# mikeferguson/ndt_2d

Measured on AMD Instinct MI355X. Metric: pose-candidates x beams scored per second, higher is better.
Workload: dtype f64

## Files before the change

experiments/asm_loop_mix.py:

```python
#!/usr/bin/env python3
import collections
import hashlib
import json
import os
import re
import subprocess
import sys
import tempfile

R = os.path.dirname(os.path.dirname(os.path.abspath(__file__)))
KERNELS = [
    ("ndt2d_match_lane.hip", "match_lane_compact_kernel", r"25match_lane_compact_kernelENS"),
    ("ndt2d_match_lane.hip", "match_lane_compact_parts_kernel", r"31match_lane_compact_parts_kernelENS"),
    ("ndt2d_match_small.hip", "match_small_kernel", r"18match_small_kernelILb1ELb1ELb1EEE"),
    ("ndt2d_poses_compact.hip", "score_poses_compact_kernel", r"26score_poses_compact_kernelILi256ELb1ELb1ELb0EEE"),
]


def kernel_lines(path, pattern):
    out, on = [], False
    for line in open(path):
        if not on:
            if re.match(r"^_Z\w*%s\w*:" % pattern, line):
                on = True
            continue
        out.append(line)
        if line.strip().startswith("s_endpgm"):
            break
    return out


def loop_depths(lines):
    label_at = {}
    for i, line in enumerate(lines):
        m = re.match(r"^(\.LBB\d+_\d+):", line)
        if m:
            label_at[m.group(1)] = i
    depth = [0] * len(lines)
    for i, line in enumerate(lines):
        m = re.match(r"^\s+s_c?branch\w*\s+(\.LBB\d+_\d+)", line)
        if m:
            j = label_at.get(m.group(1))
            if j is not None and j <= i:
                for k in range(j, i + 1):
                    depth[k] += 1
# ... 122 lines not shown
```

experiments/lane_paths.py:

```python
#!/usr/bin/env python3
import json
import os
import sys

ROOT = os.path.dirname(os.path.dirname(os.path.abspath(__file__)))
sys.path.insert(0, ROOT)
import torch
from ndt_2d_amd import ScanMatcherNDT, synth, _capi

cfg = int(sys.argv[1]) if len(sys.argv) > 1 else 2
m = ScanMatcherNDT(0)
m.initialize("paths", **synth.matcher_params(cfg))
m.addScans(synth.map_scans(cfg))
guess, pts, _ = synth.query_scan(cfg)
n_th, n_lin, n_b = m.prepare_search(guess, pts)
if cfg == 4:
    n_th_run = (n_th + 7) // 8
    launch = lambda ptr: m.match_launch_strided(0, 8, n_th_run, scores_ptr=ptr)
else:
    n_th_run = n_th
    launch = lambda ptr: m.match_launch(0, n_th, scores_ptr=ptr)
hist = torch.zeros(256, dtype=torch.float64, device="cuda")
launch(hist.data_ptr())
m.synchronize()
hist.zero_()
torch.cuda.synchronize()
launch(hist.data_ptr())
m.synchronize()
h = hist.cpu().numpy()
names = ["items", "chunks_pretested", "beams_in_lookup_groups", "groups_with_a_live_lane", "beams_with_a_live_lane",
         "exact_evaluations", "evaluations_by_reference_index", "evaluations_with_exp", "skip_refreshes",
         "items_reduced", "single_beams"]
p1 = (n_lin + 7) // 8
out = {"what": "path counts of one search, wave-level events (experiments/lane_paths.py, -DNDT2D_LANE_PATHS build)",
       "cfg": cfg, "variant": m.last_variant(), "n_theta_run": n_th_run, "n_lin": n_lin, "beams": n_b,
       "wave_beams": n_th_run * p1 * p1 * n_b, "units": n_th_run * n_lin * n_lin * n_b,
       "build_info": _capi.build_info(),
       "counts": {n: float(h[200 + i]) for i, n in enumerate(names)}}
print(json.dumps(out, indent=1))
```

ndt_2d_amd/csrc/device/ndt2d_context.h:

```cpp
#ifndef NDT2D_CONTEXT_H_
#define NDT2D_CONTEXT_H_

#include <hip/hip_runtime.h>

#include <atomic>
#include <cmath>
#include <cstring>
#include <string>
#include <utility>
#include <vector>

#include "ndt2d_guard.h"
#include "ndt2d_hip.h"
#include "ndt2d_kernels.h"

#pragma GCC visibility push(hidden)

struct DeviceBuffer
{
  double * ptr = nullptr;
  size_t cap = 0;
  DeviceBuffer() = default;
  DeviceBuffer(const DeviceBuffer &) = delete;
  DeviceBuffer & operator=(const DeviceBuffer &) = delete;
// ... 48 lines not shown
  DeviceBuffer coarse_bits;
  int coarse_log2 = -1;
  DeviceBuffer block_bytes;
  int block_bytes_log2 = -1;
  uint32_t sparse_n = 0;
  const uint32_t * sparse_index = nullptr;
  const double * sparse_cells6 = nullptr;
  DeviceBuffer b_points, b_scans, b_offsets, b_world, b_keys, b_vals, b_temp, b_seg;
  std::vector<double> stage_scans;
  std::vector<uint32_t> stage_offsets;
  std::vector<uint32_t> stage_seen;

  DeviceBuffer beams;
  size_t n_beams = 0;
  PinnedStage stage_beams, stage_tables, stage_grid, stage_call;
  const double * beams_ptr = nullptr;
  const double * tables_ptr = nullptr;
  DeviceBuffer call_dev;

  uint64_t queued = 0, reached = 0;
  uint64_t match_pos = 0, few_pos = 0;
  double * host_res = nullptr;
  double * host_res_dev = nullptr;
  unsigned long long seq = 0;
  unsigned long long match_seq = 0;
  unsigned long long * done_words = nullptr;

  DeviceBuffer tables;
  bool tables_uploaded = false;
  size_t n_th = 0, n_lin = 0;
  double pose_x = 0.0, pose_y = 0.0;
  double dlin_absmax = 0.0;
  double patch_span = -1.0;
  double beam_rmax = 0.0;
  bool has_search = false;

  DeviceBuffer ws_match, ws_poses, record, stats, outer;
  DeviceBuffer tmp_scores, tmp_poses, tmp_noise;
  hipStream_t up_stream = nullptr, down_stream = nullptr;
  hipEvent_t pipe_up[NDT2D_PIPELINE_PIECES] = {}, pipe_scored[NDT2D_PIPELINE_PIECES] = {}, pipe_idle = nullptr;
  DeviceBuffer piece_stats;
  int pipeline_pieces = 0;
  int last_pieces = 1;
  DeviceBuffer near_list;
  DeviceBuffer scan_ranges, scan_points, scan_info;
  size_t n_scan_points = 0;

  hipEvent_t ring0[NDT2D_TIMING_HISTORY] = {}, ring1[NDT2D_TIMING_HISTORY] = {};
  uint64_t n_timed_launches = 0;
  hipEvent_t ev0 = nullptr, ev1 = nullptr;
  bool timing = true;
  bool timed = false;
  int last_kernels = 0;
  const char * last_variant = "";
  int force_variant = ndt2d::kVariantAuto;
  bool batched_only = false;
  int eigen_form = 0;

  bool match_pending = false;
  uint64_t match_launches = 0, match_fetches = 0;
  bool few_pending = false;
  unsigned long long few_seq = 0;
  size_t few_n_poses = 0;
  bool few_stats = false;
  bool sums_pending = false;
  unsigned long long sums_seq = 0;
// ... 251 lines not shown
```

ndt_2d_amd/csrc/device/ndt2d_context_search.hip:

```cpp
#include <algorithm>
#include <limits>

#include "device/ndt2d_context.h"

using namespace ndt2d_device;

namespace
{

void lattice_extent(ndt2d_context * h, const double * dlin, size_t n_lin)
{
  h->dlin_absmax = 0.0;
  h->patch_span = 0.0;
  for (size_t i = 0; i < n_lin; ++i)
  {
    if (std::fabs(dlin[i]) > h->dlin_absmax) h->dlin_absmax = std::fabs(dlin[i]);
  }
  for (size_t i = 0; i < n_lin && h->patch_span >= 0.0; i += 8)
  {
    const size_t last = i + 7 < n_lin ? i + 7 : n_lin - 1;
    for (size_t k = i; k < last; ++k)
    {
      if (!(dlin[k + 1] >= dlin[k])) h->patch_span = -1.0;
    }
    if (h->patch_span >= 0.0 && dlin[last] - dlin[i] > h->patch_span) h->patch_span = dlin[last] - dlin[i];
  }
}

}

double ndt2d_device::beam_reach(const double * beams_xy, size_t n_beams)
{
  double rmax = 0.0;
  for (size_t i = 0; i < n_beams; ++i)
  {
    const double r = std::hypot(beams_xy[2 * i], beams_xy[2 * i + 1]);
    if (r > rmax) rmax = r;
    if (std::isnan(r)) rmax = std::numeric_limits<double>::infinity();
  }
  return rmax;
}

extern "C" {

int ndt2d_set_beams(ndt2d_handle h, const double * beams_xy, size_t n_beams)
{
  NDT2D_C_TRY
  if (h == nullptr) return NDT2D_ERR_INVALID;
  if (beams_xy == nullptr || n_beams == 0 || n_beams > (1u << 20))
  {
    return fail(h, NDT2D_ERR_INVALID, "ndt2d_set_beams: bad argument");
  }
  NDT2D_HIP(h, hipSetDevice(h->device));
  int rc = ensure(h, h->beams, 2 * n_beams + 2);
  if (rc != NDT2D_OK) return rc;
  rc = stage_acquire(h, h->stage_beams, 2 * n_beams);
  if (rc != NDT2D_OK) return rc;
  std::memcpy(h->stage_beams.ptr, beams_xy, 2 * n_beams * sizeof(double));
  rc = stage_submit(h, h->stage_beams, h->beams.ptr, 2 * n_beams);
// ... 108 lines not shown
  if (h == nullptr) return NDT2D_ERR_INVALID;
  if (!h->has_grid) return fail(h, NDT2D_ERR_NO_GRID, "ndt2d_match_launch: no grid");
  if (!h->has_search || h->n_beams == 0)
  {
    return fail(h, NDT2D_ERR_STATE, "ndt2d_match_launch: set_beams/set_search first");
  }
  if (th_count == 0 || th_stride == 0 || th_first >= h->n_th ||
      (th_count - 1) > (h->n_th - 1 - th_first) / th_stride)
  {
    return fail(h, NDT2D_ERR_INVALID, "ndt2d_match_launch: bad theta range");
  }
  const size_t th_begin = th_first, th_end = th_first + th_count;
  NDT2D_TEST_MAYBE_FAIL(h, "ndt2d_match_launch");
  NDT2D_HIP(h, hipSetDevice(h->device));
  int rc = ensure(h, h->record, NDT2D_MATCH_RECORD_DOUBLES);
  if (rc != NDT2D_OK) return rc;
  if (h->bytes_job.n > 0)
  {
    hipError_t be = ndt2d::launch_sparse_bytes(h->grid, h->bytes_job, h->stream);
    if (be != hipSuccess) return fail_hip(h, be, "launch_sparse_bytes");
    h->bytes_job.n = 0;
  }

  ndt2d::MatchArgs a{};
  a.grid = h->grid;
  a.beams_xy = h->beams_ptr;
  a.n_beams = static_cast<uint32_t>(h->n_beams);
  a.dth = h->tables_ptr;
  a.cos_th = h->tables_ptr + h->n_th;
  a.sin_th = h->tables_ptr + 2 * h->n_th;
  a.dlin = h->tables_ptr + 3 * h->n_th;
  a.dlin_absmax = h->dlin_absmax;
  a.patch_span = h->patch_span;
  a.beam_rmax = h->beam_rmax;
  a.n_th = static_cast<uint32_t>(h->n_th);
  a.n_lin = static_cast<uint32_t>(h->n_lin);
  a.th_begin = static_cast<uint32_t>(th_begin);
  a.th_end = static_cast<uint32_t>(th_end);
  a.th_stride = static_cast<uint32_t>(th_stride);
  a.pose_x = h->pose_x;
  a.pose_y = h->pose_y;
  a.scores = d_scores;
  if (!(h->force_variant & (ndt2d::kVariantWave | ndt2d::kVariantLane)))
  {
    const int k = ndt2d::match_small_block_log2(a, ndt2d::poses_lds_per_block());
    if (k > 0)
    {
      if (h->block_bytes_log2 != k)
      {
        rc = ensure(h, h->block_bytes, ndt2d::grid_block_bytes_size(h->grid, static_cast<uint32_t>(k)) / 8 + 2);
        if (rc != NDT2D_OK) return rc;
        hipError_t be = ndt2d::grid_block_bytes_launch(h->grid, static_cast<uint32_t>(k),
                                                       reinterpret_cast<uint8_t *>(h->block_bytes.ptr), h->stream);
        if (be != hipSuccess) return fail_hip(h, be, "grid_block_bytes_launch");
        h->block_bytes_log2 = k;
      }
      a.grid.block_bytes = reinterpret_cast<const uint8_t *>(h->block_bytes.ptr);
      a.grid.block_bytes_log2 = static_cast<uint32_t>(k);
    }
  }
  if (!h->tables_uploaded)
  {
    a.host_tables = h->stage_tables.ptr;
    if (ndt2d::match_needs_device_tables(a, !(h->force_variant & ndt2d::kVariantWave), h->force_variant))
    {
      rc = stage_submit(h, h->stage_tables, h->tables.ptr, 3 * h->n_th + h->n_lin);
// ... 168 lines not shown
```

ndt_2d_amd/csrc/ndt2d_kernels.h:

```cpp
#ifndef NDT2D_KERNELS_H_
#define NDT2D_KERNELS_H_

#include <hip/hip_runtime.h>
#include <math.h>
#include <stddef.h>
#include <stdint.h>

inline void ndt2d_cos_sin(double t, double * c, double * s)
{
  sincos(t, s, c);
}

namespace ndt2d
{

constexpr int kCellDoubles = 6;
constexpr int kCellStrideGlobal = 8;

struct GridDesc
{
  const double * cells_lds_image;
  const double * cells_global;
  const uint32_t * occ_bits;
  const uint8_t * cell_bytes;
  const double * compact_records;
  const uint16_t * cell_rank;
  uint32_t n_occ;
  const uint8_t * block_bytes;
  uint32_t block_bytes_log2;
  uint32_t size_x, size_y, ncell;
  double cell_size;
  double inv_cell_size;
  int pow2;
  double origin_x, origin_y;
};

struct MatchArgs
{
  GridDesc grid;
  const double * beams_xy;
  uint32_t n_beams;
  const double * dth;
  const double * cos_th;
  const double * sin_th;
  const double * dlin;
  double dlin_absmax;
  double beam_rmax;
  double patch_span;
  uint32_t n_th, n_lin;
  uint32_t th_begin, th_end;
  uint32_t th_stride;
  double pose_x, pose_y;
  double * scores;
  const double * host_tables;
  uint32_t beam_parts, part_beams;
  double * part_sums;
  double * partials;
  uint32_t * next_item;
  uint32_t chunk;
};

struct PosesArgs
{
  GridDesc grid;
  const double * beams_xy;
  uint32_t n_beams;
  const double * poses_xyt;
  uint64_t n_poses;
  double * scores;
  double * partials;
  double beam_rmax;
  float screen_guard;
  const uint32_t * coarse_bits;
  uint32_t coarse_log2;
};

struct BuildArgs
{
  GridDesc grid;
  const double * points_xy;
  uint32_t n_points;
// ... 215 lines not shown
```

ndt_2d_amd/csrc/ndt2d_lane_fn.h:

```cpp
#ifndef NDT2D_LANE_FN_H_
#define NDT2D_LANE_FN_H_

#include <cmath>

#include "ndt2d_device_fn.h"

namespace ndt2d
{

namespace
{

constexpr int kPatch = 8;
#ifndef NDT2D_LANE_UNROLL
#define NDT2D_LANE_UNROLL 8
#endif
constexpr int kUnroll = NDT2D_LANE_UNROLL;
constexpr double kFracScale = 65536.0;
constexpr int kMapStride = 256;
constexpr int kMaxMapCells = 256;
constexpr uint32_t kNearUnits = 4;
constexpr double kBoxMargin = 1.0 / 1024.0;
constexpr double kTwo24 = 16777216.0;
constexpr double kTwo52 = 4503599627370496.0;
constexpr double kNearBias = kNearUnits * (kTwo24 + 1.0);
static_assert(kNearUnits == 4, "near_boundary() tests the biased fraction against 2 * kNearUnits");

struct LaneGeom
{
  int32_t pad;
  int32_t sub_log2;
  int32_t block_log2;
  double unit_scale;
  double inv_scaled;
  int32_t map_h;
  int32_t win_x0, win_y0, win_w, win_h;
  double k_min, k_max_x, k_max_y;
  int32_t no_skip;
  int32_t box_span;
};

constexpr int kMaxBoxSpan = 3;
constexpr int kMaxBlockLog2 = 3;

__device__ __forceinline__ double exponent_upper_bound(const double * rec, double x0, double x1,
                                                       double y0, double y1)
{
  const double mx = rec[0], my = rec[1], h00 = rec[2], h01 = rec[3], h11 = rec[4];
  if (!(h00 < 0.0 && h11 < 0.0 && h00 * h11 - h01 * h01 > 0.0)) return HUGE_VAL;
  const double a0 = x0 - mx, a1 = x1 - mx, b0 = y0 - my, b1 = y1 - my;
  double best;
  if (a0 <= 0.0 && a1 >= 0.0 && b0 <= 0.0 && b1 >= 0.0)
  {
    best = 0.0;
  }
  else
  {
    best = -HUGE_VAL;
    const double qa[2] = {a0, a1}, qb[2] = {b0, b1};
#pragma unroll
    for (int k = 0; k < 2; ++k)
    {
      double q0 = qa[k];
      double q1 = fmin(fmax(-h01 * q0 / h11, b0), b1);
      best = fmax(best, h00 * q0 * q0 + 2.0 * h01 * q0 * q1 + h11 * q1 * q1);
      q1 = qb[k];
      q0 = fmin(fmax(-h01 * q1 / h00, a0), a1);
      best = fmax(best, h00 * q0 * q0 + 2.0 * h01 * q0 * q1 + h11 * q1 * q1);
    }
  }
  const double am = fmax(fabs(a0), fabs(a1)), bm = fmax(fabs(b0), fabs(b1));
  const double magnitude = fabs(h00) * am * am + 2.0 * fabs(h01) * am * bm + fabs(h11) * bm * bm;
  return best + (1e-9 * magnitude + 1e-6);
}

// ... 179 lines not shown
__device__ __forceinline__ uint64_t near_boundary(uint32_t v)
{
  uint64_t lanes;
  asm("v_cmp_gt_u16_e64 %0, 8, %1" : "=s"(lanes) : "v"(v));
  return lanes;
}

__device__ __forceinline__ uint2 lds_two_dwords_at(uint32_t address)
{
  typedef const __attribute__((address_space(3), aligned(4))) uint32_t * lds_u32_ptr;
  const lds_u32_ptr p = reinterpret_cast<lds_u32_ptr>(address);
  return make_uint2(p[0], p[1]);
}

__device__ __forceinline__ bool patch_can_score(double s, int32_t span)
{
  const uint32_t lo = static_cast<uint32_t>(__double2loint(s));
  const uint32_t hi = static_cast<uint32_t>(__double2hiint(s));
  const uint32_t address = __builtin_amdgcn_perm(hi, lo, 0x0c0c0502u);
  const uint32_t base = address & ~3u;
  const uint32_t shift = address & 3u;
  uint32_t any = 0;
#pragma unroll
  for (int r = 0; r <= kMaxBoxSpan; ++r)
  {
    if (r <= span)
    {
      const uint2 w = lds_two_dwords_at(base + static_cast<uint32_t>(r) * kMapStride);
      any |= __builtin_amdgcn_alignbyte(w.y, w.x, shift);
    }
  }
  const uint32_t columns = span >= 3 ? 0xfcfcfcfcu : (0xfcfcfcfcu >> (8 * (3 - span)));
  return (any & columns) != 0u;
}

__device__ __forceinline__ double lds_record_exponent(uint32_t cells_address, uint32_t idx,
                                                      double px, double py)
{
  typedef const __attribute__((address_space(3), aligned(16))) double * lds_double_ptr;
  const lds_double_ptr rec = reinterpret_cast<lds_double_ptr>(
    __umul24(idx, static_cast<uint32_t>(kCellDoubles * sizeof(double))) + cells_address);
  return record_exponent(rec[0], rec[1], rec[2], rec[3], rec[4], px, py);
}

struct SkipState
{
  double skip_below;
  uint32_t skip_level;
};

__device__ __forceinline__ SkipState skip_state(double sum, int32_t no_skip)
{
  SkipState s;
  if (no_skip)
  {
    s.skip_below = -HUGE_VAL;
    s.skip_level = 0;
    return s;
  }
  s.skip_below = negligible_below(sum);
  const int32_t l = static_cast<int32_t>(ceil(s.skip_below)) + 63;
  s.skip_level = static_cast<uint32_t>(min(max(l, 1), 63)) << 2;
  return s;
}

template <int U, bool POW2, bool LDS_RECORDS, bool SCALAR_ROWS = true, bool COMPACT = false>
// ... 145 lines not shown
  }
  if (coarse_map && block_log2 > 0)
  {
    const int32_t cells = 1 << block_log2;
    geo->win_w += geo->win_x0 & (cells - 1);
    geo->win_h += geo->win_y0 & (cells - 1);
    geo->win_x0 &= ~(cells - 1);
    geo->win_y0 &= ~(cells - 1);
  }
  geo->pad = pad;
  geo->block_log2 = block_log2;
  const size_t grid_bytes = static_cast<size_t>(args.grid.ncell + 1) * kCellDoubles * sizeof(double);
  const bool records_fit = grid_bytes + kMapStride * need_h <= lds_per_block;
  const uint64_t p1 = (args.n_lin + kPatch - 1) / kPatch;
  const bool small_search = static_cast<uint64_t>(args.n_th) * p1 * p1 < 4096;
  int sub_log2 = (small_search || coarse_map || block_log2 > 0) ? 0 : 2;
  for (; sub_log2 > 0; --sub_log2)
  {
    const uint64_t w = need_w << sub_log2, h = need_h << sub_log2;
    if (w > kMaxMapCells || h > kMaxMapCells) continue;
    const size_t bytes = static_cast<size_t>(kMapStride) * h + (records_fit ? grid_bytes : 0);
    if (bytes <= lds_per_block) break;
  }
  geo->sub_log2 = sub_log2;
  geo->unit_scale = kFracScale * static_cast<double>(1 << sub_log2) / static_cast<double>(1 << block_log2);
  geo->inv_scaled = args.grid.inv_cell_size * geo->unit_scale;
  geo->map_h = static_cast<int32_t>((need_h << sub_log2) >> block_log2);
  const double reach_units = (lin_cells + 1.0) * geo->unit_scale;
  geo->k_min = reach_units;
  geo->k_max_x = static_cast<double>(need_w - 1) * geo->unit_scale - reach_units;
  geo->k_max_y = static_cast<double>(need_h - 1) * geo->unit_scale - reach_units;
  *map_bytes = static_cast<size_t>(kMapStride) * geo->map_h;
  geo->box_span = -1;
  if (args.patch_span >= 0.0)
  {
    const double span_units = std::ceil(args.patch_span * args.grid.inv_cell_size * geo->unit_scale) + 2.0;
    const double sub_cells = std::floor((65535.0 + span_units) / 65536.0);
    if (sub_cells <= static_cast<double>(kMaxBoxSpan)) geo->box_span = static_cast<int32_t>(sub_cells);
  }
  return true;
}

}

}

#endif
```

ndt_2d_amd/csrc/ndt2d_match_lane.hip:

```cpp
#include <cmath>
#include <cstdlib>

#include <type_traits>

#include "ndt2d_lane_fn.h"

namespace ndt2d
{

namespace
{

constexpr uint32_t kDynamicItemsFromBeams = 256;
constexpr int kLaneThreads = 1024;
constexpr int kLaneThreadsSmall = 256;
#ifndef NDT2D_LANE_THREADS_COMPACT
#define NDT2D_LANE_THREADS_COMPACT 768
#endif
constexpr int kLaneThreadsCompact = NDT2D_LANE_THREADS_COMPACT;
#define NDT2D_LANE_COMPACT_WAVES_PER_EU (NDT2D_LANE_THREADS_COMPACT / 128)

__global__ void __launch_bounds__(256) outer_table_kernel(const MatchArgs a, double4 * outer,
                                                          uint8_t * map_out, const LaneGeom geo)
{
// ... 11 lines not shown
        continue;
      }
      const int32_t sub = 1 << geo.sub_log2;
      const int32_t cx = (mx >> geo.sub_log2) - geo.pad + geo.win_x0;
      const int32_t cy = (my >> geo.sub_log2) - geo.pad + geo.win_y0;
      map_out[i] = sub_cell_byte(g, cx, cy, mx & (sub - 1), my & (sub - 1), geo.sub_log2);
    }
  }

  if (blockIdx.x == 0 && threadIdx.x < kItemShards) a.next_item[threadIdx.x * kItemShardStride] = 0u;
  const uint64_t n = static_cast<uint64_t>(a.th_end - a.th_begin) * a.n_beams;
  for (uint64_t i = static_cast<uint64_t>(blockIdx.x) * 256 + threadIdx.x; i < n;
       i += static_cast<uint64_t>(gridDim.x) * 256)
  {
    const uint32_t t = static_cast<uint32_t>(i / a.n_beams);
    const uint32_t b = static_cast<uint32_t>(i - static_cast<uint64_t>(t) * a.n_beams);
    const uint32_t ith = a.th_begin + t * a.th_stride;
    const double ct = a.cos_th[ith];
    const double st = a.sin_th[ith];
    const double2 p = reinterpret_cast<const double2 *>(a.beams_xy)[b];
    double4 o;
    o.x = p.x * ct - p.y * st + a.pose_x;
    o.y = p.x * st + p.y * ct + a.pose_y;
    double kx = ((o.x - a.grid.origin_x) * a.grid.inv_cell_size + (geo.pad - geo.win_x0)) * geo.unit_scale;
    double ky = ((o.y - a.grid.origin_y) * a.grid.inv_cell_size + (geo.pad - geo.win_y0)) * geo.unit_scale;
    kx = !(kx >= geo.k_min) ? geo.k_min : (kx > geo.k_max_x ? geo.k_max_x : kx);
    ky = !(ky >= geo.k_min) ? geo.k_min : (ky > geo.k_max_y ? geo.k_max_y : ky);
    o.z = kTwo52 + (rint(ky) * kTwo24 + rint(kx)) + kNearBias;
    o.w = 0.0;
    outer[i] = o;
  }
}

__device__ __forceinline__ void item_place(uint32_t item, uint32_t patches, uint32_t patches_1d,
                                           uint32_t th_mid, uint32_t & t, uint32_t & pxi, uint32_t & pyi)
{
  const uint32_t rank = item / patches;
  const uint32_t p = item - rank * patches;
  t = (rank & 1u) ? th_mid + (rank + 1u) / 2u : th_mid - rank / 2u;
  pxi = p / patches_1d;
  pyi = p - pxi * patches_1d;
}

__device__ __forceinline__ double packed_offset(double dx, double dy, double inv_scaled)
{
  return rint(dy * inv_scaled) * kTwo24 + rint(dx * inv_scaled);
}

__device__ __forceinline__ double no_index_here()
{
  static_assert(kNoIndex == 1.0e308, "the literal below is 1.0e308");
  uint32_t lo, hi;
  asm volatile("v_mov_b32 %0, 0x85ebc8a0\n\tv_mov_b32 %1, 0x7fe1ccf3" : "=v"(lo), "=v"(hi));
  return __hiloint2double(static_cast<int>(hi), static_cast<int>(lo));
}

template <int THREADS, bool POW2, bool LDS_RECORDS, bool DYNAMIC_ITEMS, bool COMPACT, bool PARTS = false>
__device__ __forceinline__ void match_lane_body(
  const MatchArgs & a, const double4 * __restrict__ outer, const uint8_t * __restrict__ map_image,
  const LaneGeom & geo)
{
  extern __shared__ __align__(16) double lds[];
  const GridDesc & g = a.grid;
#if defined(NDT2D_LANE_HIST) || defined(NDT2D_LANE_PATHS)
  if (blockIdx.x == 0 && threadIdx.x == 0) g_lane_hist = a.scores;
#endif
  uint8_t * lds_map = reinterpret_cast<uint8_t *>(lds);
  const uint32_t map_bytes = static_cast<uint32_t>(geo.map_h) * kMapStride;
  const uint32_t rank_bytes = COMPACT ? compact_rank_bytes(g.ncell) : 0u;
  double * lds_cells = lds + (map_bytes + rank_bytes) / sizeof(double);

  if (COMPACT)
  {
    const uint4 * src_rank = reinterpret_cast<const uint4 *>(g.cell_rank);
    uint4 * dst_rank = reinterpret_cast<uint4 *>(lds_map + map_bytes + kRankLead);
    for (uint32_t i = threadIdx.x; i < (rank_bytes - kRankLead) / 16; i += THREADS) dst_rank[i] = src_rank[i];
    if (threadIdx.x == 0)
    {
      reinterpret_cast<uint16_t *>(lds_map + map_bytes + kRankLead)[-1] = static_cast<uint16_t>(g.n_occ);
    }
    const uint32_t n2 = (g.n_occ + 1) * kCellDoubles / 2;
    const double2 * src = reinterpret_cast<const double2 *>(g.compact_records);
    double2 * dst = reinterpret_cast<double2 *>(lds_cells);
    for (uint32_t i = threadIdx.x; i < n2; i += THREADS) dst[i] = src[i];
  }
  else if (LDS_RECORDS)
  {
    stage_grid_to_lds(g, lds_cells);
  }
  {
    const uint32_t n16 = static_cast<uint32_t>(kMapStride) * geo.map_h / 16;
    const uint4 * src = reinterpret_cast<const uint4 *>(map_image);
    uint4 * dst = reinterpret_cast<uint4 *>(lds_map);
    for (uint32_t i = threadIdx.x; i < n16; i += THREADS) dst[i] = src[i];
  }
  __syncthreads();

#ifdef NDT2D_LANE_TRACE
  const unsigned long long trace_t0 = wall_clock64();
  unsigned long long trace_last = trace_t0, trace_max = 0, trace_last_start = trace_t0;
  uint32_t trace_items = 0, trace_prev_item = 0, trace_flagged = 0;
#endif
  LaneCtx c;
  c.rank_address = map_bytes + (COMPACT ? kRankLead : 0u);
  c.lds_cells_address = map_bytes + rank_bytes;
  c.sub_log2 = static_cast<uint32_t>(geo.sub_log2);
  c.exact_index = geo.block_log2 > 0 ? 1u : 0u;
  c.idx_bias = static_cast<uint32_t>(geo.pad - geo.win_y0) * g.size_x +
               static_cast<uint32_t>(geo.pad - geo.win_x0);
  c.size_x = g.size_x;

  const uint32_t lane = threadIdx.x & (kWave - 1);
  const uint32_t wave = __builtin_amdgcn_readfirstlane(threadIdx.x >> 6);
  const uint32_t n_lin = a.n_lin;
  const uint32_t patches_1d = (n_lin + kPatch - 1) / kPatch;
  const uint32_t patches = patches_1d * patches_1d;
  const uint32_t n_items = (a.th_end - a.th_begin) * patches * (PARTS ? a.beam_parts : 1u);
  constexpr uint32_t kLaneWaves = THREADS / kWave;
  const uint32_t n_workers = gridDim.x * kLaneWaves;
  const uint32_t worker = wave * gridDim.x + blockIdx.x;
  const uint64_t per_theta = static_cast<uint64_t>(n_lin) * n_lin;
  const uint32_t th_mid = (a.th_end - a.th_begin - 1u) / 2u;
  const uint32_t home_shard = blockIdx.x % kItemShards;
  const double inv_scaled = geo.inv_scaled;

  double best_s = 0.0;
  double best_i = kNoIndex;
  double acc[10];
#pragma unroll
  for (int k = 0; k < 10; ++k) acc[k] = 0.0;
  for (uint32_t item = worker; item < n_items;)
  {
    uint32_t t, pxi, pyi;
#ifdef NDT2D_LANE_TRACE
    {
      const unsigned long long now = wall_clock64();
      if (trace_items > 0 && now - trace_last > trace_max) trace_max = now - trace_last;
      if (trace_items > 0 && a.scores != nullptr && lane == 0)
      {
        a.scores[5 * 8192 + 150000 + trace_prev_item] = static_cast<double>(now - trace_last);
        a.scores[5 * 8192 + 300000 + trace_prev_item] = static_cast<double>(trace_flagged);
      }
      trace_flagged = 0;
      trace_prev_item = item;
      trace_last = now;
      trace_last_start = now;
      ++trace_items;
      if (a.scores != nullptr && lane == 0) a.scores[5 * 8192 + item] = static_cast<double>(now);
    }
#endif
    const uint32_t whole_item = PARTS ? item / a.beam_parts : item;
    const uint32_t part = PARTS ? item - whole_item * a.beam_parts : 0u;
    item_place(whole_item, patches, patches_1d, th_mid, t, pxi, pyi);
    uint32_t lane_here = lane;
    asm volatile("" : "+v"(lane_here));
    const uint32_t ix = pxi * kPatch + (lane_here >> 3);
    const uint32_t iy = pyi * kPatch + (lane_here & 7);
    const double dx = a.dlin[min(ix, n_lin - 1)];
    const double dy = a.dlin[min(iy, n_lin - 1)];
    const double dxy = packed_offset(dx, dy, inv_scaled);
    const double4 * __restrict__ row = outer + static_cast<size_t>(t) * a.n_beams;

    double sum = 0.0;
    SkipState skip = skip_state(0.0, geo.no_skip);
    NDT2D_PATH(200, 1);
    const double dxy_corner = __hiloint2double(__builtin_amdgcn_readfirstlane(__double2hiint(dxy)),
                                               __builtin_amdgcn_readfirstlane(__double2loint(dxy)));
    const uint32_t beams_begin = PARTS ? part * a.part_beams : 0u;
    const uint32_t beams_end = PARTS ? min(beams_begin + a.part_beams, a.n_beams) : a.n_beams;
    for (uint32_t b0 = beams_begin; b0 < beams_end; b0 += kWave)
    {
      uint64_t can_score = ~0ull;
      if (geo.box_span >= 0)
      {
        const double k = row[min(b0 + lane, a.n_beams - 1u)].z;
        can_score = __builtin_amdgcn_ballot_w64(patch_can_score(k + dxy_corner, geo.box_span));
        NDT2D_PATH(201, 1);
      }
#ifdef NDT2D_LANE_TRACE
      trace_flagged += static_cast<uint32_t>(__popcll(can_score));
#endif
      const uint32_t chunk_end = min(b0 + static_cast<uint32_t>(kWave), beams_end);
      uint32_t b = b0;
      for (; b + kUnroll <= chunk_end; b += kUnroll, can_score >>= kUnroll)
      {
        if ((can_score & ((1ull << kUnroll) - 1ull)) == 0ull) continue;
        double4 o[kUnroll];
#pragma unroll
        for (int u = 0; u < kUnroll; ++u) o[u] = row[b + u];
        __builtin_amdgcn_s_setprio(3);
        lane_beams<kUnroll, POW2, LDS_RECORDS, true, COMPACT>(g, c, o, dx, dy, dxy, sum, skip, geo.no_skip);
        __builtin_amdgcn_s_setprio(0);
      }
      for (; b < chunk_end; ++b, can_score >>= 1)
      {
        if ((can_score & 1ull) == 0ull) continue;
        const double4 one[1] = {row[b]};
        lane_beams<1, POW2, LDS_RECORDS, true, COMPACT>(g, c, one, dx, dy, dxy, sum, skip, geo.no_skip);
      }
    }

    if (PARTS)
    {
      a.part_sums[static_cast<size_t>(item) * kWave + lane] = sum;
      uint32_t next = n_items;
      if (lane == kWave - 1)
      {
        for (uint32_t tried = 0; tried < kItemShards && next >= n_items; ++tried)
        {
          const uint32_t shard = (home_shard + tried) % kItemShards;
          const uint32_t k = atomicAdd(a.next_item + shard * kItemShardStride, 1u);
          const uint64_t candidate = static_cast<uint64_t>(n_workers) + static_cast<uint64_t>(k) * kItemShards + shard;
          if (candidate < n_items) next = static_cast<uint32_t>(candidate);
        }
      }
      item = static_cast<uint32_t>(__builtin_amdgcn_readlane(static_cast<int>(next), kWave - 1));
      continue;
    }
    uint32_t lane_again = lane;
    asm volatile("" : "+v"(lane_again));
    const uint32_t ix_e = pxi * kPatch + (lane_again >> 3);
    const uint32_t iy_e = pyi * kPatch + (lane_again & 7);
    if ((ix_e < n_lin) & (iy_e < n_lin))
    {
      const uint32_t ix = ix_e, iy = iy_e;
      const double score = -sum;
      const uint64_t local = static_cast<uint64_t>(t) * per_theta + static_cast<uint64_t>(ix) * n_lin + iy;
      const double flat = static_cast<double>(
        static_cast<uint64_t>(a.th_begin + t * a.th_stride) * per_theta + static_cast<uint64_t>(ix) * n_lin + iy);
      if (DYNAMIC_ITEMS)
      {
        if (score < best_s)
        {
          best_s = score;
          best_i = flat;
        }
      }
      else if (score < 0.0)
      {
        merge_best(score, flat, best_s, best_i);
      }
      const double dt = a.dth[a.th_begin + t * a.th_stride];
      acc[0] += (dx * dx) * score;
      acc[1] += (dx * dy) * score;
      acc[2] += (dx * dt) * score;
      acc[3] += (dy * dy) * score;
      acc[4] += (dy * dt) * score;
      acc[5] += (dt * dt) * score;
      acc[6] += dx * score;
      acc[7] += dy * score;
      acc[8] += dt * score;
      acc[9] += score;
#if !defined(NDT2D_LANE_HIST) && !defined(NDT2D_LANE_TRACE) && !defined(NDT2D_LANE_PATHS)
      if (a.scores != nullptr) a.scores[local] = score;
#endif
    }
// ... 33 lines not shown
#pragma unroll
    for (int k = 0; k < 10; ++k) acc[k] = 0.0;
  }
#ifdef NDT2D_LANE_TRACE
  if (a.scores != nullptr && lane == 0)
  {
    const unsigned long long now = wall_clock64();
    if (trace_items > 0 && now - trace_last > trace_max) trace_max = now - trace_last;
    if (trace_items > 0) a.scores[5 * 8192 + 150000 + trace_prev_item] = static_cast<double>(now - trace_last);
    if (trace_items > 0) a.scores[5 * 8192 + 300000 + trace_prev_item] = static_cast<double>(trace_flagged);
    a.scores[5 * worker] = static_cast<double>(trace_t0);
    a.scores[5 * worker + 1] = static_cast<double>(now);
    a.scores[5 * worker + 2] = static_cast<double>(trace_items);
    a.scores[5 * worker + 3] = static_cast<double>(trace_max);
    a.scores[5 * worker + 4] = static_cast<double>(trace_last_start);
  }
#endif
  if (!DYNAMIC_ITEMS)
  {
    wave_best_to_last_lane(best_s, best_i);
#pragma unroll
    for (int k = 0; k < 10; ++k) acc[k] = wave_sum_to_last_lane(acc[k]);
    if (lane == kWave - 1)
    {
      double * out = a.partials + static_cast<size_t>(worker) * kRecord;
      out[0] = best_s;
      out[1] = best_i;
#pragma unroll
      for (int k = 0; k < 10; ++k) out[2 + k] = acc[k];
    }
  }
}

template <int THREADS, bool POW2, bool LDS_RECORDS, bool DYNAMIC_ITEMS>
__global__ void __launch_bounds__(THREADS) match_lane_kernel(
  const MatchArgs a, const double4 * __restrict__ outer, const uint8_t * __restrict__ map_image,
  const LaneGeom geo)
{
  match_lane_body<THREADS, POW2, LDS_RECORDS, DYNAMIC_ITEMS, false>(a, outer, map_image, geo);
}

__global__ void __launch_bounds__(kLaneThreadsCompact) __attribute__((amdgpu_waves_per_eu(NDT2D_LANE_COMPACT_WAVES_PER_EU)))
match_lane_compact_kernel(const MatchArgs a, const double4 * __restrict__ outer,
                          const uint8_t * __restrict__ map_image, const LaneGeom geo)
{
  match_lane_body<kLaneThreadsCompact, true, true, true, true>(a, outer, map_image, geo);
}

template <bool POW2>
__global__ void __launch_bounds__(kLaneThreadsCompact) __attribute__((amdgpu_waves_per_eu(NDT2D_LANE_COMPACT_WAVES_PER_EU)))
match_lane_gather6_kernel(const MatchArgs a, const double4 * __restrict__ outer,
                          const uint8_t * __restrict__ map_image, const LaneGeom geo)
{
  match_lane_body<kLaneThreadsCompact, POW2, false, true, false>(a, outer, map_image, geo);
}

__global__ void __launch_bounds__(kLaneThreadsCompact) __attribute__((amdgpu_waves_per_eu(NDT2D_LANE_COMPACT_WAVES_PER_EU)))
match_lane_compact_parts_kernel(const MatchArgs a, const double4 * __restrict__ outer,
                                const uint8_t * __restrict__ map_image, const LaneGeom geo)
{
  match_lane_body<kLaneThreadsCompact, true, true, true, true, true>(a, outer, map_image, geo);
}

template <bool POW2>
__global__ void __launch_bounds__(kLaneThreadsCompact) __attribute__((amdgpu_waves_per_eu(NDT2D_LANE_COMPACT_WAVES_PER_EU)))
match_lane_gather6_parts_kernel(const MatchArgs a, const double4 * __restrict__ outer,
                                const uint8_t * __restrict__ map_image, const LaneGeom geo)
{
  match_lane_body<kLaneThreadsCompact, POW2, false, true, false, true>(a, outer, map_image, geo);
}

__global__ void __launch_bounds__(256) match_lane_combine_kernel(const MatchArgs a)
{
  const uint32_t lane = threadIdx.x & (kWave - 1);
  const uint32_t n_lin = a.n_lin;
  const uint32_t patches_1d = (n_lin + kPatch - 1) / kPatch;
  const uint32_t patches = patches_1d * patches_1d;
  const uint32_t n_items = (a.th_end - a.th_begin) * patches;
  const uint32_t item = blockIdx.x * 4u + (threadIdx.x >> 6);
  if (item >= n_items) return;
  const uint32_t th_mid = (a.th_end - a.th_begin - 1u) / 2u;
  uint32_t t, pxi, pyi;
  item_place(item, patches, patches_1d, th_mid, t, pxi, pyi);
  const uint32_t ix = pxi * kPatch + (lane >> 3);
  const uint32_t iy = pyi * kPatch + (lane & 7);
  const bool valid = (ix < n_lin) & (iy < n_lin);
  const double * p = a.part_sums + static_cast<size_t>(item) * a.beam_parts * kWave + lane;
// ... 138 lines not shown
  const bool dynamic_items = args.n_beams >= kDynamicItemsFromBeams;
  const uint32_t p1 = (args.n_lin + kPatch - 1) / kPatch;
  const uint64_t n_items = static_cast<uint64_t>(args.th_end - args.th_begin) * p1 * p1;

  const uint64_t n_outer = static_cast<uint64_t>(args.th_end - args.th_begin) * args.n_beams;
  uint32_t oblocks = static_cast<uint32_t>((n_outer + 255) / 256);
  if (oblocks > 4096) oblocks = 4096;
  if (oblocks < 64) oblocks = 64;
  uint8_t * map_image = reinterpret_cast<uint8_t *>(outer + n_outer * 4);
  uint32_t part_beams = 0;
  uint32_t beam_parts = dynamic_items ? lane_beam_parts(args, &part_beams) : 1u;
  args.part_sums = outer + n_outer * 4 + static_cast<size_t>(kMapStride) * kMaxMapCells / sizeof(double);

  const char * knob_rec = std::getenv("NDT2D_LANE_RECORDS");
  const bool lds_records = lane_records_in_lds(args, map_bytes, lds_per_block) &&
                           !(knob_rec != nullptr && knob_rec[0] == 'g');
  size_t lds_bytes =
    map_bytes +
    (lds_records ? static_cast<size_t>(args.grid.ncell + 1) * kCellDoubles * sizeof(double) : 0);
  const size_t compact_bytes =
    compact_rank_bytes(args.grid.ncell) +
    (static_cast<size_t>(args.grid.n_occ) + 1) * kCellDoubles * sizeof(double);
  const char * knob = std::getenv("NDT2D_LANE_COMPACT");
  const bool compact_possible = dynamic_items && pow2_grid(args) && lds_records && args.grid.n_occ > 0 &&
                                args.grid.compact_records != nullptr &&
                                2 * (map_bytes + compact_bytes) <= lds_per_block &&
                                !(knob != nullptr && knob[0] == '0');
  const char * knob6 = std::getenv("NDT2D_LANE_GATHER6");
  const bool gather6_possible = dynamic_items && !lds_records && 2 * map_bytes <= lds_per_block &&
                                !(knob6 != nullptr && knob6[0] == '0');
  if (!(compact_possible || gather6_possible)) beam_parts = 1;
  args.beam_parts = beam_parts;
  args.part_beams = part_beams;
  const uint64_t n_sub_items = n_items * beam_parts;

  const bool small = beam_parts == 1 && n_items <= static_cast<uint64_t>(cus) * (kLaneThreadsSmall / kWave);
  const uint32_t waves_per_block = (small ? kLaneThreadsSmall : kLaneThreads) / kWave;
  uint32_t blocks = static_cast<uint32_t>((n_items + waves_per_block - 1) / waves_per_block);
  uint32_t max_blocks = static_cast<uint32_t>(cus);
  if (max_blocks * waves_per_block > max_workers) max_blocks = max_workers / waves_per_block;
  if (blocks > max_blocks) blocks = max_blocks;
  if (blocks == 0) blocks = 1;
  const bool compact = !small && compact_possible;
  const bool gather6 = !compact && !small && gather6_possible;
  if (records_mode_out != nullptr)
  {
    *records_mode_out = (compact ? 2 : (lds_records ? 1 : 0)) | (geo.block_log2 > 0 ? 4 : 0);
  }
  if (compact || gather6)
  {
    lds_bytes = compact ? map_bytes + compact_bytes : map_bytes;
    const uint32_t wpb = kLaneThreadsCompact / kWave;
    blocks = static_cast<uint32_t>((n_sub_items + wpb - 1) / wpb);
    uint32_t cap = 2 * static_cast<uint32_t>(cus);
    if (cap * wpb > max_workers) cap = max_workers / wpb;
    if (blocks > cap) blocks = cap;
    if (blocks == 0) blocks = 1;
  }
  hipLaunchKernelGGL(outer_table_kernel, dim3(oblocks), dim3(256), 0, stream, args,
                     reinterpret_cast<double4 *>(outer), map_image, geo);
  hipError_t e = hipGetLastError();
  if (e != hipSuccess) return e;
  if (ev_after_pre_kernel != nullptr)
  {
    e = hipEventRecord(ev_after_pre_kernel, stream);
    if (e != hipSuccess) return e;
  }
  auto launch = [&](auto kernel, int threads) -> hipError_t {
    const hipError_t e2 = prepare_absolute_lds_kernel(reinterpret_cast<const void *>(kernel), lds_bytes);
    if (e2 != hipSuccess) return e2;
    hipLaunchKernelGGL(kernel, dim3(blocks), dim3(threads), lds_bytes, stream, args,
                       reinterpret_cast<const double4 *>(outer),
                       static_cast<const uint8_t *>(map_image), geo);
    return hipGetLastError();
  };
  const bool pow2 = args.grid.pow2 != 0;
  auto pick = [&](auto threads_tag) -> hipError_t {
    constexpr int T = decltype(threads_tag)::value;
    auto with_items = [&](auto dyn_tag) -> hipError_t {
      constexpr bool D = decltype(dyn_tag)::value;
      return lds_records ? (pow2 ? launch(match_lane_kernel<T, true, true, D>, T)
                                 : launch(match_lane_kernel<T, false, true, D>, T))
                         : (pow2 ? launch(match_lane_kernel<T, true, false, D>, T)
                                 : launch(match_lane_kernel<T, false, false, D>, T));
    };
    return dynamic_items ? with_items(std::true_type{}) : with_items(std::false_type{});
  };
  if (beam_parts > 1)
  {
    e = compact ? launch(match_lane_compact_parts_kernel, kLaneThreadsCompact)
                : (pow2 ? launch(match_lane_gather6_parts_kernel<true>, kLaneThreadsCompact)
                        : launch(match_lane_gather6_parts_kernel<false>, kLaneThreadsCompact));
    if (e == hipSuccess)
    {
      hipLaunchKernelGGL(match_lane_combine_kernel, dim3(static_cast<uint32_t>((n_items + 3) / 4)), dim3(256),
                         0, stream, args);
      e = hipGetLastError();
    }
  }
  else if (compact)
  {
    e = launch(match_lane_compact_kernel, kLaneThreadsCompact);
  }
  else if (gather6)
  {
    e = pow2 ? launch(match_lane_gather6_kernel<true>, kLaneThreadsCompact)
             : launch(match_lane_gather6_kernel<false>, kLaneThreadsCompact);
  }
  else
  {
    e = small ? pick(std::integral_constant<int, kLaneThreadsSmall>{})
              : pick(std::integral_constant<int, kLaneThreads>{});
  }
  if (parts_out != nullptr) *parts_out = beam_parts;
  if (n_workers_out != nullptr)
  {
    *n_workers_out = dynamic_items ? static_cast<uint32_t>(n_items) : blocks * waves_per_block;
  }
  return e;
}

}
```

Measured before the change: 3038 billion.

## Tile ragged lane-grid edges with long thin strips instead of padded 8x8 patches

When n_lin is not a multiple of the 8-wide patch (remainder 1-4), the edge rows and columns are covered by strips of 16-64 by 1-4 cells, so each wave fills its 64 lanes instead of running mostly-idle padded 8x8 edge patches. Host-side search setup computes per-strip offset spans, and a new strip_can_score map-occupancy pretest covers wider boxes for these tiles. Strips are only enabled for the unsplit dynamic-item kernel forms. This cuts wasted lanes on edge tiles, at the cost of more kernel template variants and a heavier pretest for strip tiles.

Measured after the change: 3084 billion (median of 6 runs). +1.5%, better.

```diff
diff --git a/experiments/asm_loop_mix.py b/experiments/asm_loop_mix.py
--- a/experiments/asm_loop_mix.py
+++ b/experiments/asm_loop_mix.py
@@ -10,7 +10,7 @@
 
 R = os.path.dirname(os.path.dirname(os.path.abspath(__file__)))
 KERNELS = [
-    ("ndt2d_match_lane.hip", "match_lane_compact_kernel", r"25match_lane_compact_kernelENS"),
+    ("ndt2d_match_lane.hip", "match_lane_compact_kernel", r"25match_lane_compact_kernelILb1EEE"),
     ("ndt2d_match_lane.hip", "match_lane_compact_parts_kernel", r"31match_lane_compact_parts_kernelENS"),
     ("ndt2d_match_small.hip", "match_small_kernel", r"18match_small_kernelILb1ELb1ELb1EEE"),
     ("ndt2d_poses_compact.hip", "score_poses_compact_kernel", r"26score_poses_compact_kernelILi256ELb1ELb1ELb0EEE"),
diff --git a/experiments/lane_paths.py b/experiments/lane_paths.py
--- a/experiments/lane_paths.py
+++ b/experiments/lane_paths.py
@@ -31,10 +31,10 @@
 names = ["items", "chunks_pretested", "beams_in_lookup_groups", "groups_with_a_live_lane", "beams_with_a_live_lane",
          "exact_evaluations", "evaluations_by_reference_index", "evaluations_with_exp", "skip_refreshes",
          "items_reduced", "single_beams"]
-p1 = (n_lin + 7) // 8
+items = float(h[200])
 out = {"what": "path counts of one search, wave-level events (experiments/lane_paths.py, -DNDT2D_LANE_PATHS build)",
        "cfg": cfg, "variant": m.last_variant(), "n_theta_run": n_th_run, "n_lin": n_lin, "beams": n_b,
-       "wave_beams": n_th_run * p1 * p1 * n_b, "units": n_th_run * n_lin * n_lin * n_b,
+       "wave_beams": items * n_b, "units": n_th_run * n_lin * n_lin * n_b,
        "build_info": _capi.build_info(),
        "counts": {n: float(h[200 + i]) for i, n in enumerate(names)}}
 print(json.dumps(out, indent=1))
diff --git a/ndt_2d_amd/csrc/device/ndt2d_context.h b/ndt_2d_amd/csrc/device/ndt2d_context.h
--- a/ndt_2d_amd/csrc/device/ndt2d_context.h
+++ b/ndt_2d_amd/csrc/device/ndt2d_context.h
@@ -104,6 +104,7 @@
   double pose_x = 0.0, pose_y = 0.0;
   double dlin_absmax = 0.0;
   double patch_span = -1.0;
+  double strip_span_long = 0.0, strip_span_short = 0.0;
   double beam_rmax = 0.0;
   bool has_search = false;
 
diff --git a/ndt_2d_amd/csrc/device/ndt2d_context_search.hip b/ndt_2d_amd/csrc/device/ndt2d_context_search.hip
--- a/ndt_2d_amd/csrc/device/ndt2d_context_search.hip
+++ b/ndt_2d_amd/csrc/device/ndt2d_context_search.hip
@@ -2,6 +2,7 @@
 #include <limits>
 
 #include "device/ndt2d_context.h"
+#include "ndt2d_lane_fn.h"
 
 using namespace ndt2d_device;
 
@@ -25,6 +26,20 @@
     }
     if (h->patch_span >= 0.0 && dlin[last] - dlin[i] > h->patch_span) h->patch_span = dlin[last] - dlin[i];
   }
+  h->strip_span_long = h->strip_span_short = 0.0;
+  uint32_t long_log2 = 0;
+  if (!ndt2d::lane_strip_shape(static_cast<uint32_t>(n_lin), &long_log2)) return;
+  for (size_t k = 0; k + 1 < n_lin; ++k)
+  {
+    if (!(dlin[k + 1] >= dlin[k])) return;
+  }
+  const size_t group = static_cast<size_t>(1) << long_log2;
+  for (size_t i = 0; i < n_lin; i += group)
+  {
+    const size_t last = i + group - 1 < n_lin ? i + group - 1 : n_lin - 1;
+    if (dlin[last] - dlin[i] > h->strip_span_long) h->strip_span_long = dlin[last] - dlin[i];
+  }
+  h->strip_span_short = dlin[n_lin - 1] - dlin[n_lin / 8 * 8];
 }
 
 }
@@ -199,6 +214,8 @@
   a.dlin = h->tables_ptr + 3 * h->n_th;
   a.dlin_absmax = h->dlin_absmax;
   a.patch_span = h->patch_span;
+  a.strip_span_long = h->strip_span_long;
+  a.strip_span_short = h->strip_span_short;
   a.beam_rmax = h->beam_rmax;
   a.n_th = static_cast<uint32_t>(h->n_th);
   a.n_lin = static_cast<uint32_t>(h->n_lin);
diff --git a/ndt_2d_amd/csrc/ndt2d_kernels.h b/ndt_2d_amd/csrc/ndt2d_kernels.h
--- a/ndt_2d_amd/csrc/ndt2d_kernels.h
+++ b/ndt_2d_amd/csrc/ndt2d_kernels.h
@@ -47,6 +47,7 @@
   double dlin_absmax;
   double beam_rmax;
   double patch_span;
+  double strip_span_long, strip_span_short;
   uint32_t n_th, n_lin;
   uint32_t th_begin, th_end;
   uint32_t th_stride;
diff --git a/ndt_2d_amd/csrc/ndt2d_lane_fn.h b/ndt_2d_amd/csrc/ndt2d_lane_fn.h
--- a/ndt_2d_amd/csrc/ndt2d_lane_fn.h
+++ b/ndt_2d_amd/csrc/ndt2d_lane_fn.h
@@ -38,9 +38,80 @@
   double k_min, k_max_x, k_max_y;
   int32_t no_skip;
   int32_t box_span;
+  int32_t strips;
+  int32_t strip_span_long, strip_span_short;
 };
 
 constexpr int kMaxBoxSpan = 3;
+constexpr int kMaxStripSpan = 7;
+
+struct LaneTiling
+{
+  uint32_t row;
+  uint32_t core;
+  uint32_t long_log2;
+  uint32_t tiles_x;
+  uint32_t per_theta;
+};
+
+__host__ __device__ inline bool lane_strip_shape(uint32_t n_lin, uint32_t * long_log2)
+{
+  const uint32_t rem = n_lin % kPatch;
+  if (rem == 0 || rem > 4) return false;
+  *long_log2 = rem == 1 ? 6u : (rem == 2 ? 5u : 4u);
+  return true;
+}
+
+__host__ __device__ inline LaneTiling lane_tiling(uint32_t n_lin, bool strips)
+{
+  LaneTiling t;
+  uint32_t long_log2 = 3;
+  if (strips && lane_strip_shape(n_lin, &long_log2))
+  {
+    const uint32_t full = n_lin / kPatch;
+    const uint32_t round_up = (1u << long_log2) - 1u;
+    t.row = full;
+    t.core = full * full;
+    t.long_log2 = long_log2;
+    t.tiles_x = (n_lin + round_up) >> long_log2;
+    t.per_theta = t.core + t.tiles_x + ((full * kPatch + round_up) >> long_log2);
+    return t;
+  }
+  t.row = (n_lin + kPatch - 1) / kPatch;
+  t.core = t.row * t.row;
+  t.long_log2 = 3;
+  t.tiles_x = 0;
+  t.per_theta = t.core;
+  return t;
+}
+
+__host__ __device__ inline void lane_tile(const LaneTiling & t, uint32_t n_lin, uint32_t p, uint32_t & x0,
+                                          uint32_t & y0, uint32_t & h_log2, uint32_t & x_end)
+{
+  if (p < t.core)
+  {
+    const uint32_t pxi = p / t.row;
+    x0 = pxi * kPatch;
+    y0 = (p - pxi * t.row) * kPatch;
+    h_log2 = 3;
+    x_end = n_lin;
+    return;
+  }
+  const uint32_t q = p - t.core;
+  if (q < t.tiles_x)
+  {
+    x0 = t.row * kPatch;
+    y0 = q << t.long_log2;
+    h_log2 = t.long_log2;
+    x_end = n_lin;
+    return;
+  }
+  x0 = (q - t.tiles_x) << t.long_log2;
+  y0 = t.row * kPatch;
+  h_log2 = 6u - t.long_log2;
+  x_end = t.row * kPatch;
+}
+
 constexpr int kMaxBlockLog2 = 3;
 
 __device__ __forceinline__ double exponent_upper_bound(const double * rec, double x0, double x1,
@@ -286,6 +357,30 @@
   }
   const uint32_t columns = span >= 3 ? 0xfcfcfcfcu : (0xfcfcfcfcu >> (8 * (3 - span)));
   return (any & columns) != 0u;
+}
+
+__device__ __forceinline__ bool strip_can_score(double s, int32_t span_x, int32_t span_y)
+{
+  typedef const __attribute__((address_space(3), aligned(4))) uint32_t * lds_u32_ptr;
+  const uint32_t lo = static_cast<uint32_t>(__double2loint(s));
+  const uint32_t hi = static_cast<uint32_t>(__double2hiint(s));
+  const uint32_t address = __builtin_amdgcn_perm(hi, lo, 0x0c0c0502u);
+  const uint32_t base = address & ~3u;
+  const uint32_t shift = address & 3u;
+  uint32_t any_lo = 0, any_hi = 0;
+#pragma unroll
+  for (int r = 0; r <= kMaxStripSpan; ++r)
+  {
+    if (r <= span_y)
+    {
+      const lds_u32_ptr p = reinterpret_cast<lds_u32_ptr>(base + static_cast<uint32_t>(r) * kMapStride);
+      const uint32_t w0 = p[0], w1 = p[1], w2 = p[2];
+      any_lo |= __builtin_amdgcn_alignbyte(w1, w0, shift);
+      any_hi |= __builtin_amdgcn_alignbyte(w2, w1, shift);
+    }
+  }
+  const uint64_t columns = 0xfcfcfcfcfcfcfcfcull >> (8 * (kMaxStripSpan - span_x));
+  return ((any_lo & static_cast<uint32_t>(columns)) | (any_hi & static_cast<uint32_t>(columns >> 32))) != 0u;
 }
 
 __device__ __forceinline__ double lds_record_exponent(uint32_t cells_address, uint32_t idx,
@@ -497,12 +592,30 @@
   geo->k_max_y = static_cast<double>(need_h - 1) * geo->unit_scale - reach_units;
   *map_bytes = static_cast<size_t>(kMapStride) * geo->map_h;
   geo->box_span = -1;
+  const auto span_sub_cells = [&](double span) {
+    const double span_units = std::ceil(span * args.grid.inv_cell_size * geo->unit_scale) + 2.0;
+    return std::floor((65535.0 + span_units) / 65536.0);
+  };
   if (args.patch_span >= 0.0)
   {
-    const double span_units = std::ceil(args.patch_span * args.grid.inv_cell_size * geo->unit_scale) + 2.0;
-    const double sub_cells = std::floor((65535.0 + span_units) / 65536.0);
+    const double sub_cells = span_sub_cells(args.patch_span);
     if (sub_cells <= static_cast<double>(kMaxBoxSpan)) geo->box_span = static_cast<int32_t>(sub_cells);
   }
+  geo->strips = 0;
+  geo->strip_span_long = geo->strip_span_short = 0;
+  uint32_t long_log2 = 0;
+  if (geo->box_span >= 0 && lane_strip_shape(args.n_lin, &long_log2) && args.strip_span_long > 0.0 &&
+      args.strip_span_short >= 0.0)
+  {
+    const double sub_long = span_sub_cells(args.strip_span_long);
+    const double sub_short = span_sub_cells(args.strip_span_short);
+    if (sub_long <= static_cast<double>(kMaxStripSpan) && sub_short <= static_cast<double>(kMaxStripSpan))
+    {
+      geo->strips = 1;
+      geo->strip_span_long = static_cast<int32_t>(sub_long);
+      geo->strip_span_short = static_cast<int32_t>(sub_short);
+    }
+  }
   return true;
 }
 
diff --git a/ndt_2d_amd/csrc/ndt2d_match_lane.hip b/ndt_2d_amd/csrc/ndt2d_match_lane.hip
--- a/ndt_2d_amd/csrc/ndt2d_match_lane.hip
+++ b/ndt_2d_amd/csrc/ndt2d_match_lane.hip
@@ -67,12 +67,19 @@
   }
 }
 
+__device__ __forceinline__ void item_step(uint32_t item, uint32_t patches, uint32_t th_mid, uint32_t & t,
+                                          uint32_t & p)
+{
+  const uint32_t rank = item / patches;
+  p = item - rank * patches;
+  t = (rank & 1u) ? th_mid + (rank + 1u) / 2u : th_mid - rank / 2u;
+}
+
 __device__ __forceinline__ void item_place(uint32_t item, uint32_t patches, uint32_t patches_1d,
                                            uint32_t th_mid, uint32_t & t, uint32_t & pxi, uint32_t & pyi)
 {
-  const uint32_t rank = item / patches;
-  const uint32_t p = item - rank * patches;
-  t = (rank & 1u) ? th_mid + (rank + 1u) / 2u : th_mid - rank / 2u;
+  uint32_t p;
+  item_step(item, patches, th_mid, t, p);
   pxi = p / patches_1d;
   pyi = p - pxi * patches_1d;
 }
@@ -90,7 +97,8 @@
   return __hiloint2double(static_cast<int>(hi), static_cast<int>(lo));
 }
 
-template <int THREADS, bool POW2, bool LDS_RECORDS, bool DYNAMIC_ITEMS, bool COMPACT, bool PARTS = false>
+template <int THREADS, bool POW2, bool LDS_RECORDS, bool DYNAMIC_ITEMS, bool COMPACT, bool PARTS = false,
+          bool STRIPS = false>
 __device__ __forceinline__ void match_lane_body(
   const MatchArgs & a, const double4 * __restrict__ outer, const uint8_t * __restrict__ map_image,
   const LaneGeom & geo)
@@ -148,8 +156,9 @@
   const uint32_t lane = threadIdx.x & (kWave - 1);
   const uint32_t wave = __builtin_amdgcn_readfirstlane(threadIdx.x >> 6);
   const uint32_t n_lin = a.n_lin;
-  const uint32_t patches_1d = (n_lin + kPatch - 1) / kPatch;
-  const uint32_t patches = patches_1d * patches_1d;
+  static_assert(!STRIPS || (DYNAMIC_ITEMS && !PARTS), "strip tiles: the unsplit dynamic-item forms only");
+  const LaneTiling tiling = lane_tiling(n_lin, STRIPS);
+  const uint32_t patches = tiling.per_theta;
   const uint32_t n_items = (a.th_end - a.th_begin) * patches * (PARTS ? a.beam_parts : 1u);
   constexpr uint32_t kLaneWaves = THREADS / kWave;
   const uint32_t n_workers = gridDim.x * kLaneWaves;
@@ -166,7 +175,7 @@
   for (int k = 0; k < 10; ++k) acc[k] = 0.0;
   for (uint32_t item = worker; item < n_items;)
   {
-    uint32_t t, pxi, pyi;
+    uint32_t t, p;
 #ifdef NDT2D_LANE_TRACE
     {
       const unsigned long long now = wall_clock64();
@@ -186,12 +195,25 @@
 #endif
     const uint32_t whole_item = PARTS ? item / a.beam_parts : item;
     const uint32_t part = PARTS ? item - whole_item * a.beam_parts : 0u;
-    item_place(whole_item, patches, patches_1d, th_mid, t, pxi, pyi);
+    item_step(whole_item, patches, th_mid, t, p);
+    uint32_t x0, y0, h_log2, x_end;
+    if (STRIPS)
+    {
+      lane_tile(tiling, n_lin, p, x0, y0, h_log2, x_end);
+    }
+    else
+    {
+      x0 = p / tiling.row * kPatch;
+      y0 = (p - p / tiling.row * tiling.row) * kPatch;
+      h_log2 = 3;
+      x_end = n_lin;
+    }
+    const bool strip_tile = STRIPS && p >= tiling.core;
     uint32_t lane_here = lane;
     asm volatile("" : "+v"(lane_here));
-    const uint32_t ix = pxi * kPatch + (lane_here >> 3);
-    const uint32_t iy = pyi * kPatch + (lane_here & 7);
-    const double dx = a.dlin[min(ix, n_lin - 1)];
+    const uint32_t ix = x0 + (lane_here >> h_log2);
+    const uint32_t iy = y0 + (lane_here & ((1u << h_log2) - 1u));
+    const double dx = a.dlin[min(ix, x_end - 1)];
     const double dy = a.dlin[min(iy, n_lin - 1)];
     const double dxy = packed_offset(dx, dy, inv_scaled);
     const double4 * __restrict__ row = outer + static_cast<size_t>(t) * a.n_beams;
@@ -209,7 +231,17 @@
       if (geo.box_span >= 0)
       {
         const double k = row[min(b0 + lane, a.n_beams - 1u)].z;
-        can_score = __builtin_amdgcn_ballot_w64(patch_can_score(k + dxy_corner, geo.box_span));
+        if (strip_tile)
+        {
+          const bool along_x = h_log2 < 3u;
+          can_score = __builtin_amdgcn_ballot_w64(
+            strip_can_score(k + dxy_corner, along_x ? geo.strip_span_long : geo.strip_span_short,
+                            along_x ? geo.strip_span_short : geo.strip_span_long));
+        }
+        else
+        {
+          can_score = __builtin_amdgcn_ballot_w64(patch_can_score(k + dxy_corner, geo.box_span));
+        }
         NDT2D_PATH(201, 1);
       }
 #ifdef NDT2D_LANE_TRACE
@@ -254,9 +286,9 @@
     }
     uint32_t lane_again = lane;
     asm volatile("" : "+v"(lane_again));
-    const uint32_t ix_e = pxi * kPatch + (lane_again >> 3);
-    const uint32_t iy_e = pyi * kPatch + (lane_again & 7);
-    if ((ix_e < n_lin) & (iy_e < n_lin))
+    const uint32_t ix_e = x0 + (lane_again >> h_log2);
+    const uint32_t iy_e = y0 + (lane_again & ((1u << h_log2) - 1u));
+    if ((ix_e < x_end) & (iy_e < n_lin))
     {
       const uint32_t ix = ix_e, iy = iy_e;
       const double score = -sum;
@@ -356,27 +388,28 @@
   }
 }
 
-template <int THREADS, bool POW2, bool LDS_RECORDS, bool DYNAMIC_ITEMS>
+template <int THREADS, bool POW2, bool LDS_RECORDS, bool DYNAMIC_ITEMS, bool STRIPS = false>
 __global__ void __launch_bounds__(THREADS) match_lane_kernel(
   const MatchArgs a, const double4 * __restrict__ outer, const uint8_t * __restrict__ map_image,
   const LaneGeom geo)
 {
-  match_lane_body<THREADS, POW2, LDS_RECORDS, DYNAMIC_ITEMS, false>(a, outer, map_image, geo);
-}
-
+  match_lane_body<THREADS, POW2, LDS_RECORDS, DYNAMIC_ITEMS, false, false, STRIPS>(a, outer, map_image, geo);
+}
+
+template <bool STRIPS>
 __global__ void __launch_bounds__(kLaneThreadsCompact) __attribute__((amdgpu_waves_per_eu(NDT2D_LANE_COMPACT_WAVES_PER_EU)))
 match_lane_compact_kernel(const MatchArgs a, const double4 * __restrict__ outer,
                           const uint8_t * __restrict__ map_image, const LaneGeom geo)
 {
-  match_lane_body<kLaneThreadsCompact, true, true, true, true>(a, outer, map_image, geo);
-}
-
-template <bool POW2>
+  match_lane_body<kLaneThreadsCompact, true, true, true, true, false, STRIPS>(a, outer, map_image, geo);
+}
+
+template <bool POW2, bool STRIPS>
 __global__ void __launch_bounds__(kLaneThreadsCompact) __attribute__((amdgpu_waves_per_eu(NDT2D_LANE_COMPACT_WAVES_PER_EU)))
 match_lane_gather6_kernel(const MatchArgs a, const double4 * __restrict__ outer,
                           const uint8_t * __restrict__ map_image, const LaneGeom geo)
 {
-  match_lane_body<kLaneThreadsCompact, POW2, false, true, false>(a, outer, map_image, geo);
+  match_lane_body<kLaneThreadsCompact, POW2, false, true, false, false, STRIPS>(a, outer, map_image, geo);
 }
 
 __global__ void __launch_bounds__(kLaneThreadsCompact) __attribute__((amdgpu_waves_per_eu(NDT2D_LANE_COMPACT_WAVES_PER_EU)))
@@ -581,11 +614,15 @@
   if (!(compact_possible || gather6_possible)) beam_parts = 1;
   args.beam_parts = beam_parts;
   args.part_beams = part_beams;
-  const uint64_t n_sub_items = n_items * beam_parts;
+  if (!(dynamic_items && beam_parts == 1)) geo.strips = 0;
+  const bool strips = geo.strips != 0;
+  const uint64_t n_tiles =
+    static_cast<uint64_t>(args.th_end - args.th_begin) * lane_tiling(args.n_lin, geo.strips != 0).per_theta;
+  const uint64_t n_sub_items = beam_parts > 1 ? n_items * beam_parts : n_tiles;
 
   const bool small = beam_parts == 1 && n_items <= static_cast<uint64_t>(cus) * (kLaneThreadsSmall / kWave);
   const uint32_t waves_per_block = (small ? kLaneThreadsSmall : kLaneThreads) / kWave;
-  uint32_t blocks = static_cast<uint32_t>((n_items + waves_per_block - 1) / waves_per_block);
+  uint32_t blocks = static_cast<uint32_t>((n_tiles + waves_per_block - 1) / waves_per_block);
   uint32_t max_blocks = static_cast<uint32_t>(cus);
   if (max_blocks * waves_per_block > max_workers) max_blocks = max_workers / waves_per_block;
   if (blocks > max_blocks) blocks = max_blocks;
@@ -626,14 +663,16 @@
   const bool pow2 = args.grid.pow2 != 0;
   auto pick = [&](auto threads_tag) -> hipError_t {
     constexpr int T = decltype(threads_tag)::value;
-    auto with_items = [&](auto dyn_tag) -> hipError_t {
+    auto with_items = [&](auto dyn_tag, auto strips_tag) -> hipError_t {
       constexpr bool D = decltype(dyn_tag)::value;
-      return lds_records ? (pow2 ? launch(match_lane_kernel<T, true, true, D>, T)
-                                 : launch(match_lane_kernel<T, false, true, D>, T))
-                         : (pow2 ? launch(match_lane_kernel<T, true, false, D>, T)
-                                 : launch(match_lane_kernel<T, false, false, D>, T));
+      constexpr bool S = decltype(strips_tag)::value;
+      return lds_records ? (pow2 ? launch(match_lane_kernel<T, true, true, D, S>, T)
+                                 : launch(match_lane_kernel<T, false, true, D, S>, T))
+                         : (pow2 ? launch(match_lane_kernel<T, true, false, D, S>, T)
+                                 : launch(match_lane_kernel<T, false, false, D, S>, T));
     };
-    return dynamic_items ? with_items(std::true_type{}) : with_items(std::false_type{});
+    if (!dynamic_items) return with_items(std::false_type{}, std::false_type{});
+    return strips ? with_items(std::true_type{}, std::true_type{}) : with_items(std::true_type{}, std::false_type{});
   };
   if (beam_parts > 1)
   {
@@ -649,12 +688,15 @@
   }
   else if (compact)
   {
-    e = launch(match_lane_compact_kernel, kLaneThreadsCompact);
+    e = strips ? launch(match_lane_compact_kernel<true>, kLaneThreadsCompact)
+               : launch(match_lane_compact_kernel<false>, kLaneThreadsCompact);
   }
   else if (gather6)
   {
-    e = pow2 ? launch(match_lane_gather6_kernel<true>, kLaneThreadsCompact)
-             : launch(match_lane_gather6_kernel<false>, kLaneThreadsCompact);
+    e = pow2 ? (strips ? launch(match_lane_gather6_kernel<true, true>, kLaneThreadsCompact)
+                       : launch(match_lane_gather6_kernel<true, false>, kLaneThreadsCompact))
+             : (strips ? launch(match_lane_gather6_kernel<false, true>, kLaneThreadsCompact)
+                       : launch(match_lane_gather6_kernel<false, false>, kLaneThreadsCompact));
   }
   else
   {
@@ -664,7 +706,8 @@
   if (parts_out != nullptr) *parts_out = beam_parts;
   if (n_workers_out != nullptr)
   {
-    *n_workers_out = dynamic_items ? static_cast<uint32_t>(n_items) : blocks * waves_per_block;
+    *n_workers_out = dynamic_items ? static_cast<uint32_t>(beam_parts > 1 ? n_items : n_tiles)
+                                   : blocks * waves_per_block;
   }
   return e;
 }
```
